# AditMeh/torch-distributed-sandbox

Hardware: AMD Instinct MI355X
Metric: images/sec (whole node), 3000x3000 MNIST ConvNet DDP at 1/2/4/8 MI355X (higher is better)
Workload: dtype fp32 (conv2 fwd+dgrad+wgrad: TF32-class -- one fp16 MFMA per product, both operands rounded to 11 significant bits = TF32's significand, exact power-of-two range scaling, fp32 accumulate: the arithmetic of the reference's default cuDNN TF32 convolutions; conv1 fwd+wgrad: bf16x3 split MFMA (~2^-16)

## Files before the change

torch_distributed_sandbox_amd/csrc/kernels/conv2_fwd2.hip:

```cpp
#include <cstdlib>

#include "bn_finalize.h"
#include "conv2_common.h"
#include "launchers.h"
#include "pooled_layout.h"

namespace tds {

constexpr int F2_TH = 8, F2_TC = 16;
constexpr int F2_SR = F2_TH + 4, F2_SC = F2_TC + 4;
constexpr int F2_REC = F2_SR * F2_SC;
constexpr int F2_THREADS = 256;
constexpr int F2_PGROUPS = 8;
constexpr int F2_PPLANE = F2_PGROUPS * 32 * 32;
constexpr int F2_PBUF = F2_PPLANE;
constexpr int F2_WG = 3;
constexpr int F2_PXREC = 32 * 2 + 16;
constexpr int F2_STAGE = F2_TH * F2_TC * F2_PXREC;
constexpr int F2_OFF_S = 2 * F2_PBUF;
constexpr int F2_YSTAGE = 32 * 32 * 4 + 32 * 2 * 4;
constexpr int F2_OFF_Y = F2_OFF_S + 2 * F2_STAGE;
constexpr int F2_LDS = F2_OFF_Y + 2 * F2_YSTAGE;
constexpr int F2_DMA_PER_WAVE = F2_PGROUPS / (F2_THREADS / 64);
static_assert(F2_LDS % 16 == 0, "LDS carve");
static_assert(F2_WG * F2_LDS <= 160 * 1024, "workgroups per CU");

__device__ __attribute__((aligned(16))) uint32_t g_f2_zero[4] = {0u, 0u, 0u, 0u};

struct F2Tile {
  int b, r0, c0;
};

template <int DIAG, int WV>
__device__ __forceinline__ void f2_dma(const uint4* __restrict__ p1, const F2Tile& x, int P, char* buf, int lane) {
  if constexpr (DIAG == 3) return;
  const char* base = reinterpret_cast<const char*>(p1) + (((int64_t)x.b * P + x.r0 - 2) * P + (x.c0 - 2)) * 32;
#pragma unroll
  for (int j = 0; j < F2_DMA_PER_WAVE; ++j) {
    const int rg = WV * F2_DMA_PER_WAVE + j;
    const int px = rg * 32 + (lane >> 1), half = lane & 1;
    const int rr = px / F2_SC, cc = px - rr * F2_SC;
    const int gr = x.r0 - 2 + rr, gc = x.c0 - 2 + cc;
    const bool ok = px < F2_REC && gr >= 0 && gr < P && gc >= 0 && gc < P;
    const char* src = ok ? base + ((int64_t)rr * P + cc) * 32 + half * 16 : reinterpret_cast<const char*>(g_f2_zero);
    __builtin_amdgcn_global_load_lds(src, (__attribute__((address_space(3))) void*)(buf + rg * 1024), 16, 0, 0);
  }
}

template <int DIAG>
__device__ __forceinline__ void f2_compute(const char* buf, const f32x4 (&W)[13], f32x4 (&acc)[4], int RH, int lane) {
  constexpr int DEPTH = 4;
  const int li = lane & 15, g = lane >> 4;
  const int boff = (g & 1) * 16;
  const char* ph = buf;
#pragma unroll
  for (int o = 0; o < 4; ++o) acc[o] = f32x4{0.f, 0.f, 0.f, 0.f};
  s16x8 ah[DEPTH];
  auto load_a = [&](int i) {
    const int grp = i >> 3, R = i & 7;
    int rec;
    if (grp < 2) {
      rec = (4 * RH + R) * F2_SC + li + 2 * grp + (g >> 1);
    } else {
      int row = 4 * RH + R + (g >> 1);
      if (row > F2_SR - 1) row = F2_SR - 1;
      rec = row * F2_SC + li + 4;
    }
    ah[i % DEPTH] = lds8<DIAG>(ph + rec * 32 + boff);
  };
#pragma unroll
  for (int i = 0; i < DEPTH - 1; ++i) load_a(i);
#pragma unroll
  for (int i = 0; i < 24; ++i) {
    if (i + DEPTH - 1 < 24) load_a(i + DEPTH - 1);
    __builtin_amdgcn_sched_barrier(0);
    const int grp = i >> 3, R = i & 7, cur = i % DEPTH;
    if (grp < 2) {
#pragma unroll
      for (int ky = 0; ky < 5; ++ky) {
        const int o = R - ky;
        if (o >= 0 && o < 4)
          acc[o] = mmaw<DIAG>(ah[cur], __builtin_bit_cast(s16x8, W[2 * ky + grp]), acc[o]);
      }
    } else {
#pragma unroll
      for (int kp = 0; kp < 3; ++kp) {
        const int o = R - 2 * kp;
        if (o >= 0 && o < 4)
          acc[o] = mmaw<DIAG>(ah[cur], __builtin_bit_cast(s16x8, W[10 + kp]), acc[o]);
      }
    }
  }
}

__device__ __forceinline__ int f2_stage_off(int row, int px, int chunk) {
  return (row * F2_TC + px) * F2_PXREC + chunk * 16;
}

__device__ __forceinline__ int f2_ystage_off(int co, int e) { return co * 32 + ((((e >> 2) ^ co) & 7) << 2) + (e & 3); }

__device__ __forceinline__ float f2_ext4(float a, float b, float c, float d, bool neg) {
  const float mx = __builtin_elementwise_maximum(__builtin_elementwise_maximum(a, b), __builtin_elementwise_maximum(c, d));
  const float mn = __builtin_elementwise_minimum(__builtin_elementwise_minimum(a, b), __builtin_elementwise_minimum(c, d));
  return neg ? mn : mx;
}

typedef float f2v __attribute__((ext_vector_type(2)));
template <bool EDGE, bool PLAIN>
__device__ __forceinline__ void f2_stage(const f32x4 (&acc)[4], const F2Tile& x, char* stage, float* ystage, int P,
                                         int RH, int NT, int lane, float bco, float inv, float ksc, bool neg, bool zg,
                                         f2v& s_acc, f2v& q_acc, uint32_t& ymx, uint32_t* __restrict__ a2) {
  const int li = lane & 15, g = lane >> 4;
  const int co = 16 * NT + li;
  float ymf = 0.f;
  uint32_t h[4][4];
#pragma unroll
  for (int o = 0; o < 4; ++o)
#pragma unroll
    for (int r = 0; r < 4; ++r) h[o][r] = f16_bits(acc[o][r] * ksc);
#pragma unroll
  for (int o = 0; o < 4; ++o) {
    const int row = 4 * RH + o;
    const bool rok = !EDGE || x.r0 + row < P;
    if constexpr (EDGE) {
#pragma unroll
      for (int r = 0; r < 4; ++r) {
        const float v = acc[o][r];
        if (rok && x.c0 + 4 * g + r < P) {
          s_acc.x += v;
          q_acc.x += v * v;
          ymx = max(ymx, __float_as_uint(v) & 0x7fffffffu);
        }
      }
    } else {
#pragma unroll
      for (int r = 0; r < 4; r += 2) {
        const f2v v = {acc[o][r], acc[o][r + 1]};
        s_acc += v;
        q_acc = __builtin_elementwise_fma(v, v, q_acc);
        ymf = __builtin_elementwise_maximum(ymf, __builtin_elementwise_maximum(fabsf(v.x), fabsf(v.y)));
      }
    }
  }
  if constexpr (!EDGE) ymx = max(ymx, __float_as_uint(ymf));
  uint64_t cb0[4], cb1[4];
#pragma unroll
  for (int i = 0; i < 2; ++i) {
    uint32_t e[2];
#pragma unroll
    for (int j = 0; j < 2; ++j) {
      const float v0 = acc[2 * i][2 * j], v1 = acc[2 * i][2 * j + 1], v2 = acc[2 * i + 1][2 * j];
      const float v3 = acc[2 * i + 1][2 * j + 1];
      float m;
      if constexpr (PLAIN)
        m = __builtin_elementwise_maximum(__builtin_elementwise_maximum(v0, v1), __builtin_elementwise_maximum(v2, v3));
      else
        m = zg ? v0 : f2_ext4(v0, v1, v2, v3, neg);
      e[j] = f16_bits(m * ksc);
      const uint64_t b0 = __builtin_amdgcn_ballot_w64(v0 == m), b1 = __builtin_amdgcn_ballot_w64(v1 == m),
                     b2 = __builtin_amdgcn_ballot_w64(v2 == m);
      cb0[2 * i + j] = ~b0 & (b1 | ~b2);
      cb1[2 * i + j] = ~b0 & ~b1;
    }
    *reinterpret_cast<uint2*>(ystage + f2_ystage_off(co, (2 * RH + i) * 8 + 2 * g)) = make_uint2(e[0], e[1]);
  }
  {
    uint32_t* ab = reinterpret_cast<uint32_t*>(ystage + 32 * 32);
    const bool upper = g >= 2;
    const uint32_t psel = (g & 1) ? 0x07060302u : 0x05040100u;
    if (li == 0) {
#pragma unroll
      for (int sl = 0; sl < 4; ++sl) {
        const uint32_t w0 = upper ? (uint32_t)(cb0[sl] >> 32) : (uint32_t)cb0[sl];
        const uint32_t w1 = upper ? (uint32_t)(cb1[sl] >> 32) : (uint32_t)cb1[sl];
        ab[((2 * RH + (sl >> 1)) * 8 + 2 * g + (sl & 1)) * 2 + NT] = __builtin_amdgcn_perm(w1, w0, psel);
      }
    }
  }
#pragma unroll
  for (int o = 0; o < 4; ++o)
#pragma unroll
    for (int r = 0; r < 4; ++r)
      *reinterpret_cast<unsigned short*>(stage + (((4 * RH + o) * F2_TC + 4 * g + r) * F2_PXREC) + co * 2) =
          (unsigned short)h[o][r];
}

__device__ __forceinline__ void f2_store_ya(const float* ystage, const F2Tile& x, unsigned short* __restrict__ ya,
                                            const PBGeom& pg) {
  const int tr = x.r0 / F2_TH, tc = x.c0 / F2_TC;
  if (tr >= pg.Q4 || tc >= pg.Q8) return;
  const int e = threadIdx.x, co = e >> 3, part = e & 7;
  const uint4 v = *reinterpret_cast<const uint4*>(ystage + f2_ystage_off(co, part * 4));
  st_stream(reinterpret_cast<uint2*>(ya + ((((int64_t)x.b * 32 + co) * pg.Q4 + tr) * pg.Q8 + tc) * 32 + part * 4),
            make_uint2(__builtin_amdgcn_perm(v.y, v.x, 0x05040100u), __builtin_amdgcn_perm(v.w, v.z, 0x05040100u)));
}

__device__ __forceinline__ void f2_store_a2(const float* ystage, const F2Tile& x, uint32_t* __restrict__ a2, int P) {
  const int e = threadIdx.x, Q = P >> 1;
  const int py = (x.r0 >> 1) + (e >> 3), px = (x.c0 >> 1) + (e & 7);
  if (e < 32 && py < Q && px < Q)
    st_stream(reinterpret_cast<uint2*>(a2 + (((int64_t)x.b * Q + py) * Q + px) * 2),
              reinterpret_cast<const uint2*>(ystage + 32 * 32)[e]);
}

constexpr uint64_t F2_QPX = 0xfeab6732dc894510ull;
template <int DIAG>
__device__ __forceinline__ void f2_store(const char* stage, const F2Tile& x, unsigned short* __restrict__ y2h, int P) {
  if constexpr (DIAG == 4) return;
  const int e = threadIdx.x;
  const int qpx = (int)((F2_QPX >> (4 * ((e >> 2) & 15))) & 15u);
#pragma unroll
  for (int i = 0; i < F2_TH * F2_TC * 4 / F2_THREADS; ++i) {
    const int q = e + F2_THREADS * i;
    const int row = q >> 6, px = qpx, c8 = q & 3;
    const int gr = x.r0 + row, gc = x.c0 + px;
    const uint4 v = *reinterpret_cast<const uint4*>(stage + f2_stage_off(row, px, c8));
    if (gr < P && gc < P)
      st_stream(reinterpret_cast<float4*>(y2h + (((int64_t)x.b * P + gr) * P + gc) * 32 + c8 * 8),
                __builtin_bit_cast(float4, v));
  }
}

template <int DIAG, int WV>
__device__ __forceinline__ void f2_run(const uint4* __restrict__ p1, const uint4* __restrict__ wpack,
                                       const float* __restrict__ bias, const float* __restrict__ gamma,
                                       unsigned short* __restrict__ y2, unsigned short* __restrict__ ya,
                                       uint32_t* __restrict__ a2,
                                       double* __restrict__ partial, uint32_t* __restrict__ ypart,
                                       const uint32_t* __restrict__ scales,
                                       const int* __restrict__ order, int sw, int sk, int B, int P, char* smem) {
  constexpr int NT = WV & 1, RH = WV >> 1;
  const int lane = threadIdx.x & 63, li = lane & 15;
  const int tiles_c = (P + F2_TC - 1) / F2_TC, tiles_r = (P + F2_TH - 1) / F2_TH;
  const int per_img = tiles_c * tiles_r, total = per_img * B;
  const int w = xcd_remap(blockIdx.x, gridDim.x);
  const int* __restrict__ mine = order + w * sw;
  auto decode = [&](int kk) {
    F2Tile x;
    int tr, tc;
    tile_from_order(mine, kk * sk, x.b, tr, tc);
    x.r0 = tr * F2_TH;
    x.c0 = tc * F2_TC;
    return x;
  };
  f32x4 W[13];
#pragma unroll
  for (int s = 0; s < 13; ++s) W[s] = __builtin_bit_cast(f32x4, wpack[(s * 2 + NT) * 64 + lane]);
  const float bco = bias[16 * NT + li];
  const float inv = scales != nullptr ? __uint_as_float(scales[0]) * __uint_as_float(scales[1]) : 1.f;
  const float ksc = scales != nullptr ? __uint_as_float(scales[2]) : 1.f;
  const bool neg = gamma != nullptr && gamma[16 * NT + li] < 0.f;
  const bool zg = gamma != nullptr && gamma[16 * NT + li] == 0.f;
  const bool plain = __builtin_amdgcn_readfirstlane(__builtin_amdgcn_ballot_w64(neg || zg) == 0 ? 1 : 0) != 0;
  const PBGeom pg = pb_geom(P / 2);
  float* ys = reinterpret_cast<float*>(smem + F2_OFF_Y);
  f2v s_acc = {0.f, 0.f}, q_acc = {0.f, 0.f};
  double s_d = 0.0, q_d = 0.0;
  uint32_t ymx = 0u;
  f32x4 acc[4];
  F2Tile prev{0, 0, 0};
  bool have_prev = false;
  int t = w;
  if (t < total) f2_dma<DIAG, WV>(p1, decode(0), P, smem, lane);
  int kk = 0;
  for (; t < total; t += gridDim.x, ++kk) {
    const F2Tile cur = decode(kk);
    __syncthreads();
    if (t + (int)gridDim.x < total) f2_dma<DIAG, WV>(p1, decode(kk + 1), P, smem + ((kk + 1) & 1) * F2_PBUF, lane);
    if (have_prev) {
      f2_store<DIAG>(smem + F2_OFF_S + ((kk + 1) & 1) * F2_STAGE, prev, y2, P);
      f2_store_ya(ys + ((kk + 1) & 1) * (F2_YSTAGE / 4), prev, ya, pg);
      f2_store_a2(ys + ((kk + 1) & 1) * (F2_YSTAGE / 4), prev, a2, P);
    }
    f2_compute<DIAG>(smem + (kk & 1) * F2_PBUF, W, acc, RH, lane);
    if (cur.r0 + F2_TH <= P && cur.c0 + F2_TC <= P && plain)
      f2_stage<false, true>(acc, cur, smem + F2_OFF_S + (kk & 1) * F2_STAGE, ys + (kk & 1) * (F2_YSTAGE / 4), P, RH, NT,
                            lane, bco, inv, ksc, neg, zg, s_acc, q_acc, ymx, a2);
    else if (cur.r0 + F2_TH <= P && cur.c0 + F2_TC <= P)
      f2_stage<false, false>(acc, cur, smem + F2_OFF_S + (kk & 1) * F2_STAGE, ys + (kk & 1) * (F2_YSTAGE / 4), P, RH, NT, lane,
                      bco, inv, ksc, neg, zg, s_acc, q_acc, ymx, a2);
    else
      f2_stage<true, false>(acc, cur, smem + F2_OFF_S + (kk & 1) * F2_STAGE, ys + (kk & 1) * (F2_YSTAGE / 4), P, RH, NT, lane,
                     bco, inv, ksc, neg, zg, s_acc, q_acc, ymx, a2);
    s_d += (double)(s_acc.x + s_acc.y);
    q_d += (double)(q_acc.x + q_acc.y);
    s_acc = f2v{0.f, 0.f};
    q_acc = f2v{0.f, 0.f};
    prev = cur;
    have_prev = true;
  }
  __syncthreads();
  if (have_prev) {
    f2_store<DIAG>(smem + F2_OFF_S + ((kk - 1) & 1) * F2_STAGE, prev, y2, P);
    f2_store_ya(ys + ((kk - 1) & 1) * (F2_YSTAGE / 4), prev, ya, pg);
    f2_store_a2(ys + ((kk - 1) & 1) * (F2_YSTAGE / 4), prev, a2, P);
  }
  ymx = max(ymx, (uint32_t)__shfl_xor((int)ymx, 16, 64));
  ymx = max(ymx, (uint32_t)__shfl_xor((int)ymx, 32, 64));
  double s_sum = s_d, q_sum = q_d;
  s_sum += __shfl_xor(s_sum, 16, 64);
  s_sum += __shfl_xor(s_sum, 32, 64);
  q_sum += __shfl_xor(q_sum, 16, 64);
  q_sum += __shfl_xor(q_sum, 32, 64);
  __syncthreads();
  double* red = reinterpret_cast<double*>(smem);
  uint32_t* yred = reinterpret_cast<uint32_t*>(smem + 4 * 16 * 2 * 8);
  if (lane < 16) {
    red[(WV * 16 + li) * 2 + 0] = s_sum;
    red[(WV * 16 + li) * 2 + 1] = q_sum;
    yred[WV * 16 + li] = ymx;
  }
  __syncthreads();
  if (WV == 0 && lane < 64) {
    const int co = lane >> 1, k = lane & 1, nt = co >> 4, c16 = co & 15;
    const double v = (red[(nt * 16 + c16) * 2 + k] + red[((nt + 2) * 16 + c16) * 2 + k]) * (k ? (double)inv * inv : inv);
    st_agent(partial + ((int64_t)co * gridDim.x + blockIdx.x) * 2 + k, v);
    if (ypart != nullptr && k == 0)
      st_agent(ypart + co * gridDim.x + blockIdx.x,
               __float_as_uint(__uint_as_float(max(yred[nt * 16 + c16], yred[(nt + 2) * 16 + c16])) * inv));
  }
}

constexpr int F2_GROUP = 32;
struct F2Fin {
  uint32_t* sync;
  double* gsum;
  uint32_t* gmax;
  int64_t n;
  const float* beta;
  float eps, momentum;
  float* stats;
  float* running_mean;
  float* running_var;
  int64_t* num_batches;
  float* aff;
  uint32_t* mag;
};

__device__ __forceinline__ void f2_finalize(const F2Fin& fin, const double* __restrict__ partial,
                                            const uint32_t* __restrict__ ypart, const float* __restrict__ bias,
                                            const float* __restrict__ gamma, int* flag) {
  const int nwg = (int)gridDim.x, wg = (int)blockIdx.x, tid = (int)threadIdx.x;
  const int ng = (nwg + F2_GROUP - 1) / F2_GROUP, g = wg / F2_GROUP;
  const int w0 = g * F2_GROUP, w1 = min(nwg, w0 + F2_GROUP);
  double* part = reinterpret_cast<double*>(flag + 4);
  if (!tds_arrive(fin.sync + g, (uint32_t)(w1 - w0), flag)) return;
  const double s = wide_row_sum(partial + (int64_t)w0 * 2, w1 - w0, 64, 2, part, 2 * (int64_t)nwg);
  if (tid < 64) st_agent(fin.gsum + (int64_t)g * 64 + tid, s);
  if (ypart != nullptr && tid < 32) {
    uint32_t v[F2_GROUP];
#pragma unroll
    for (int u = 0; u < F2_GROUP; ++u) v[u] = ypart[(int64_t)tid * nwg + min(w0 + u, w1 - 1)];
    uint32_t m = 0u;
#pragma unroll
    for (int u = 0; u < F2_GROUP; ++u) m = max(m, v[u]);
    st_agent(fin.gmax + g * 32 + tid, m);
  }
  if (!tds_arrive(fin.sync + kSyncWordsPerSite - 1, (uint32_t)ng, flag)) return;
  const double sk = wide_row_sum(fin.gsum, ng, 64, 64, part);
  const uint32_t mx = wide_row_max(fin.gmax, ng, 32, 32, reinterpret_cast<uint32_t*>(part + 128));
  if (tid < 64) part[tid] = sk;
  __syncthreads();
  if (tid < 32) {
    const int co = tid;
    if (co == 0 && fin.num_batches) fin.num_batches[0] += 1;
    bn_finalize_channel(co, 32, part[co * 2], part[co * 2 + 1], fin.n, bias, fin.eps, fin.momentum, gamma, fin.beta,
                        fin.stats, fin.running_mean, fin.running_var, fin.aff);
    if (fin.mag != nullptr && ypart != nullptr) fin.mag[co] = mx;
  }
}

template <int DIAG>
__global__ __launch_bounds__(F2_THREADS, F2_WG) void conv2_fwd2_kernel(const uint4* __restrict__ p1,
                                                                   const uint4* __restrict__ wpack,
                                                                   const float* __restrict__ bias,
                                                                   const float* __restrict__ gamma,
                                                                   unsigned short* __restrict__ y2, unsigned short* __restrict__ ya,
                                                                   uint32_t* __restrict__ a2,
                                                                   double* __restrict__ partial,
                                                                   uint32_t* __restrict__ ypart,
                                                                   const uint32_t* __restrict__ scales,
                                                                   const int* __restrict__ order, int sw, int sk,
                                                                   int B, int P, F2Fin fin) {
  extern __shared__ __attribute__((aligned(16))) char smem[];
  const int wv = __builtin_amdgcn_readfirstlane(threadIdx.x >> 6);
  if (wv == 0) f2_run<DIAG, 0>(p1, wpack, bias, gamma, y2, ya, a2, partial, ypart, scales, order, sw, sk, B, P, smem);
  else if (wv == 1) f2_run<DIAG, 1>(p1, wpack, bias, gamma, y2, ya, a2, partial, ypart, scales, order, sw, sk, B, P, smem);
  else if (wv == 2) f2_run<DIAG, 2>(p1, wpack, bias, gamma, y2, ya, a2, partial, ypart, scales, order, sw, sk, B, P, smem);
  else f2_run<DIAG, 3>(p1, wpack, bias, gamma, y2, ya, a2, partial, ypart, scales, order, sw, sk, B, P, smem);
  if (fin.sync != nullptr) {
    __syncthreads();
    f2_finalize(fin, partial, ypart, bias, gamma, reinterpret_cast<int*>(smem));
  }
}

constexpr int F2I_YSTAGE = 32 * 32 * 4;
constexpr int F2I_OFF_Y = 2 * F2_PBUF;
constexpr int F2I_LDS = F2I_OFF_Y + 2 * F2I_YSTAGE;
static_assert(F2I_LDS % 16 == 0 && F2_WG * F2I_LDS <= 160 * 1024, "LDS carve");

template <bool PLAIN>
__device__ __forceinline__ void f2i_pool(const f32x4 (&acc)[4], float* ystage, int RH, int NT, int lane, float ksc,
                                         bool neg, bool zg) {
  const int li = lane & 15, g = lane >> 4;
  const int co = 16 * NT + li;
#pragma unroll
  for (int i = 0; i < 2; ++i) {
    uint32_t e[2];
#pragma unroll
    for (int j = 0; j < 2; ++j) {
      const float v0 = acc[2 * i][2 * j], v1 = acc[2 * i][2 * j + 1], v2 = acc[2 * i + 1][2 * j];
      const float v3 = acc[2 * i + 1][2 * j + 1];
      float m;
      if constexpr (PLAIN)
        m = __builtin_elementwise_maximum(__builtin_elementwise_maximum(v0, v1), __builtin_elementwise_maximum(v2, v3));
      else
        m = zg ? v0 : f2_ext4(v0, v1, v2, v3, neg);
      e[j] = f16_bits(m * ksc);
    }
    *reinterpret_cast<uint2*>(ystage + f2_ystage_off(co, (2 * RH + i) * 8 + 2 * g)) = make_uint2(e[0], e[1]);
  }
}

template <int WV>
__device__ __forceinline__ void f2i_run(const uint4* __restrict__ p1, const uint4* __restrict__ wpack,
                                        const float* __restrict__ gamma, unsigned short* __restrict__ ya,
                                        const uint32_t* __restrict__ scales, const int* __restrict__ order, int sw,
                                        int sk, int B, int P, char* smem) {
  constexpr int NT = WV & 1, RH = WV >> 1;
  const int lane = threadIdx.x & 63, li = lane & 15;
  const int tiles_c = (P + F2_TC - 1) / F2_TC, tiles_r = (P + F2_TH - 1) / F2_TH;
  const int total = tiles_c * tiles_r * B;
  const int w = xcd_remap(blockIdx.x, gridDim.x);
  const int* __restrict__ mine = order + w * sw;
  auto decode = [&](int kk) {
    F2Tile x;
    int tr, tc;
    tile_from_order(mine, kk * sk, x.b, tr, tc);
    x.r0 = tr * F2_TH;
    x.c0 = tc * F2_TC;
    return x;
  };
  f32x4 W[13];
#pragma unroll
  for (int s = 0; s < 13; ++s) W[s] = __builtin_bit_cast(f32x4, wpack[(s * 2 + NT) * 64 + lane]);
  const float ksc = scales != nullptr ? __uint_as_float(scales[2]) : 1.f;
  const bool neg = gamma != nullptr && gamma[16 * NT + li] < 0.f;
  const bool zg = gamma != nullptr && gamma[16 * NT + li] == 0.f;
  const bool plain = __builtin_amdgcn_readfirstlane(__builtin_amdgcn_ballot_w64(neg || zg) == 0 ? 1 : 0) != 0;
  const PBGeom pg = pb_geom(P / 2);
  float* ys = reinterpret_cast<float*>(smem + F2I_OFF_Y);
  f32x4 acc[4];
  F2Tile prev{0, 0, 0};
  bool have_prev = false;
  int t = w;
  if (t < total) f2_dma<0, WV>(p1, decode(0), P, smem, lane);
  int kk = 0;
  for (; t < total; t += gridDim.x, ++kk) {
    const F2Tile cur = decode(kk);
    __syncthreads();
    if (t + (int)gridDim.x < total) f2_dma<0, WV>(p1, decode(kk + 1), P, smem + ((kk + 1) & 1) * F2_PBUF, lane);
    if (have_prev) f2_store_ya(ys + ((kk + 1) & 1) * (F2I_YSTAGE / 4), prev, ya, pg);
    f2_compute<0>(smem + (kk & 1) * F2_PBUF, W, acc, RH, lane);
    if (plain)
      f2i_pool<true>(acc, ys + (kk & 1) * (F2I_YSTAGE / 4), RH, NT, lane, ksc, neg, zg);
    else
      f2i_pool<false>(acc, ys + (kk & 1) * (F2I_YSTAGE / 4), RH, NT, lane, ksc, neg, zg);
    prev = cur;
    have_prev = true;
  }
  __syncthreads();
  if (have_prev) f2_store_ya(ys + ((kk - 1) & 1) * (F2I_YSTAGE / 4), prev, ya, pg);
}

__global__ __launch_bounds__(F2_THREADS, F2_WG) void conv2_fwd2_inference_kernel(
    const uint4* __restrict__ p1, const uint4* __restrict__ wpack, const float* __restrict__ gamma,
    unsigned short* __restrict__ ya, const uint32_t* __restrict__ scales, const int* __restrict__ order, int sw, int sk,
    int B, int P) {
  extern __shared__ __attribute__((aligned(16))) char smem[];
  const int wv = __builtin_amdgcn_readfirstlane(threadIdx.x >> 6);
  if (wv == 0) f2i_run<0>(p1, wpack, gamma, ya, scales, order, sw, sk, B, P, smem);
  else if (wv == 1) f2i_run<1>(p1, wpack, gamma, ya, scales, order, sw, sk, B, P, smem);
  else if (wv == 2) f2i_run<2>(p1, wpack, gamma, ya, scales, order, sw, sk, B, P, smem);
  else f2i_run<3>(p1, wpack, gamma, ya, scales, order, sw, sk, B, P, smem);
}

}

using namespace tds;

int tds_conv2_fwd2_num_wg() { return F2_WG * tds_conv2_num_wg(); }

void tds_conv2_fwd2_tiles(int P, int* tiles_r, int* tiles_c) {
  *tiles_r = (P + F2_TH - 1) / F2_TH;
  *tiles_c = (P + F2_TC - 1) / F2_TC;
}

#ifdef TDS_DIAG
static int f2_diag_env() {
  const char* e = std::getenv("TDS_CONV2_DIAG");
  return e ? std::atoi(e) : 0;
}
#else
static int f2_diag_env() { return 0; }
#endif

int tds_conv2_fwd2_fin_doubles(int nwg) { return ((nwg + F2_GROUP - 1) / F2_GROUP) * 32 * 2; }
int tds_conv2_fwd2_fin_words(int nwg) { return ((nwg + F2_GROUP - 1) / F2_GROUP) * 32; }

void tds_conv2_fwd2_inference(const void* p1, const short* wp, const float* gamma, unsigned short* ya,
                              const uint32_t* scales, const int* order, int nwg, int sw, int sk, int B, int P,
                              hipStream_t st) {
  hipLaunchKernelGGL(conv2_fwd2_inference_kernel, dim3(nwg), dim3(F2_THREADS), F2I_LDS, st,
                     reinterpret_cast<const uint4*>(p1), reinterpret_cast<const uint4*>(wp), gamma, ya, scales, order, sw,
                     sk, B, P);
  TDS_LAUNCH_CHECK();
}

void tds_conv2_fwd2(const void* p1, const short* wp, const float* bias, const float* gamma, void* y2h, unsigned short* ya,
                    uint32_t* a2, double* partial, uint32_t* ypart, const uint32_t* scales, const int* order, int nwg, int sw, int sk,
                    int B, int P, hipStream_t st, const TdsBnFin* bn) {
  const dim3 grid(nwg), block(F2_THREADS);
  F2Fin fin{};
  if (bn != nullptr) {
    fin.sync = tds_sync_words(kSyncConv2Fwd, st);
    if (fin.sync == nullptr || (nwg + F2_GROUP - 1) / F2_GROUP > WRS_MAXL * 4) {
      tds_launch_fail("conv2_fwd2: in-launch BN2 finalize unavailable (sync words / group count)");
      return;
    }
    fin.gsum = bn->dwork;
    fin.gmax = bn->uwork;
    fin.n = (int64_t)B * P * P;
    fin.beta = bn->beta;
    fin.eps = bn->eps;
    fin.momentum = bn->momentum;
    fin.stats = bn->stats;
    fin.running_mean = bn->running_mean;
    fin.running_var = bn->running_var;
    fin.num_batches = bn->num_batches;
    fin.aff = bn->aff;
    fin.mag = bn->mag;
  }
  unsigned short* y2 = static_cast<unsigned short*>(y2h);
  const uint4* pp = reinterpret_cast<const uint4*>(p1);
  const uint4* w = reinterpret_cast<const uint4*>(wp);
  static bool lds_set = false;
  if (!lds_set) {
    (void)hipFuncSetAttribute(reinterpret_cast<const void*>(conv2_fwd2_kernel<0>),
                              hipFuncAttributeMaxDynamicSharedMemorySize, F2_LDS);
#ifdef TDS_DIAG
    (void)hipFuncSetAttribute(reinterpret_cast<const void*>(conv2_fwd2_kernel<1>), hipFuncAttributeMaxDynamicSharedMemorySize, F2_LDS);
    (void)hipFuncSetAttribute(reinterpret_cast<const void*>(conv2_fwd2_kernel<2>), hipFuncAttributeMaxDynamicSharedMemorySize, F2_LDS);
    (void)hipFuncSetAttribute(reinterpret_cast<const void*>(conv2_fwd2_kernel<3>), hipFuncAttributeMaxDynamicSharedMemorySize, F2_LDS);
    (void)hipFuncSetAttribute(reinterpret_cast<const void*>(conv2_fwd2_kernel<4>), hipFuncAttributeMaxDynamicSharedMemorySize, F2_LDS);
#endif
    lds_set = true;
  }
  switch (f2_diag_env()) {
#ifdef TDS_DIAG
    case 1: hipLaunchKernelGGL(conv2_fwd2_kernel<1>, grid, block, F2_LDS, st, pp, w, bias, gamma, y2, ya, a2, partial, ypart, scales, order, sw, sk, B, P, fin); break;
    case 2: hipLaunchKernelGGL(conv2_fwd2_kernel<2>, grid, block, F2_LDS, st, pp, w, bias, gamma, y2, ya, a2, partial, ypart, scales, order, sw, sk, B, P, fin); break;
    case 3: hipLaunchKernelGGL(conv2_fwd2_kernel<3>, grid, block, F2_LDS, st, pp, w, bias, gamma, y2, ya, a2, partial, ypart, scales, order, sw, sk, B, P, fin); break;
    case 4: hipLaunchKernelGGL(conv2_fwd2_kernel<4>, grid, block, F2_LDS, st, pp, w, bias, gamma, y2, ya, a2, partial, ypart, scales, order, sw, sk, B, P, fin); break;
#endif
    default: hipLaunchKernelGGL(conv2_fwd2_kernel<0>, grid, block, F2_LDS, st, pp, w, bias, gamma, y2, ya, a2, partial, ypart, scales, order, sw, sk, B, P, fin); break;
  }
  TDS_LAUNCH_CHECK();
}
```

Before: 2688.

## Precompute per-lane addresses and streamline tile loop in conv2 forward kernel

Hoists the per-lane DMA, staging and store offsets into a struct computed once per wave, and adds fast paths for interior tiles that skip bounds checks. Tile-order entries are decoded directly with the next entry prefetched, and the loop barrier becomes an explicit vmcnt wait plus syncthreads. The argmax bit packing moves from a single-lane loop to scalar pack and writelane instructions, and the y2h half-precision staging is split into its own function. The aim is to cut per-tile integer address arithmetic and divergent branches, at the cost of more live registers and some inline assembly that depends on the compiler placing values in scalar registers.

```diff
diff --git a/torch_distributed_sandbox_amd/csrc/kernels/conv2_fwd2.hip b/torch_distributed_sandbox_amd/csrc/kernels/conv2_fwd2.hip
--- a/torch_distributed_sandbox_amd/csrc/kernels/conv2_fwd2.hip
+++ b/torch_distributed_sandbox_amd/csrc/kernels/conv2_fwd2.hip
@@ -29,22 +29,77 @@
 
 struct F2Tile {
   int b, r0, c0;
+  bool full;
 };
 
+__device__ __forceinline__ F2Tile f2_tile(int entry, int P) {
+  F2Tile x;
+  x.b = entry >> 24;
+  x.r0 = ((entry >> 12) & 4095) * F2_TH;
+  x.c0 = (entry & 4095) * F2_TC;
+  x.full = x.r0 + F2_TH <= P && x.c0 + F2_TC <= P;
+  return x;
+}
+
+struct F2Lane {
+  uint32_t dma[F2_DMA_PER_WAVE];
+  uint32_t st_lds, st_glb;
+  uint32_t ya_lds;
+  int64_t ya_glb;
+  uint32_t a2_glb;
+};
+
+constexpr uint64_t F2_QPX = 0xfeab6732dc894510ull;
+__device__ __forceinline__ int f2_stage_off(int row, int px, int chunk);
+__device__ __forceinline__ int f2_ystage_off(int co, int e);
+
+template <int WV>
+__device__ __forceinline__ F2Lane f2_lane(int P, const PBGeom& pg, int lane) {
+  F2Lane L;
+#pragma unroll
+  for (int j = 0; j < F2_DMA_PER_WAVE; ++j) {
+    const int px = (WV * F2_DMA_PER_WAVE + j) * 32 + (lane >> 1), half = lane & 1;
+    const int rr = px / F2_SC, cc = px - rr * F2_SC;
+    L.dma[j] = px < F2_REC ? (uint32_t)((rr * P + cc) * 32 + half * 16) : 0u;
+  }
+  const int qpx = (int)((F2_QPX >> (4 * (lane >> 2))) & 15u), c8 = lane & 3;
+  L.st_lds = (uint32_t)f2_stage_off(WV, qpx, c8);
+  L.st_glb = (uint32_t)((WV * P + qpx) * 64 + c8 * 16);
+  const int co = WV * 8 + (lane >> 3), part = lane & 7;
+  L.ya_lds = (uint32_t)f2_ystage_off(co, part * 4);
+  L.ya_glb = (int64_t)co * pg.Q4 * pg.Q8 * 32 + part * 4;
+  L.a2_glb = (uint32_t)(((lane >> 3) * (P >> 1) + (lane & 7)) * 8);
+  return L;
+}
+
 template <int DIAG, int WV>
-__device__ __forceinline__ void f2_dma(const uint4* __restrict__ p1, const F2Tile& x, int P, char* buf, int lane) {
+__device__ __forceinline__ void f2_dma(const uint4* __restrict__ p1, const F2Tile& x, int P, char* buf, int lane,
+                                       const F2Lane& L) {
   if constexpr (DIAG == 3) return;
-  const char* base = reinterpret_cast<const char*>(p1) + (((int64_t)x.b * P + x.r0 - 2) * P + (x.c0 - 2)) * 32;
+  const char* base = reinterpret_cast<const char*>(p1) + ((int64_t)(x.b * P + x.r0 - 2) * P + (x.c0 - 2)) * 32;
+  if (x.r0 >= 2 && x.c0 >= 2 && x.r0 + F2_TH + 2 <= P && x.c0 + F2_TC + 2 <= P) {
+#pragma unroll
+    for (int j = 0; j < F2_DMA_PER_WAVE; ++j)
+      __builtin_amdgcn_global_load_lds(base + L.dma[j],
+                                       (__attribute__((address_space(3))) void*)(buf + (WV * F2_DMA_PER_WAVE + j) * 1024),
+                                       16, 0, 0);
+    return;
+  }
 #pragma unroll
   for (int j = 0; j < F2_DMA_PER_WAVE; ++j) {
     const int rg = WV * F2_DMA_PER_WAVE + j;
-    const int px = rg * 32 + (lane >> 1), half = lane & 1;
+    const int px = rg * 32 + (lane >> 1);
     const int rr = px / F2_SC, cc = px - rr * F2_SC;
     const int gr = x.r0 - 2 + rr, gc = x.c0 - 2 + cc;
     const bool ok = px < F2_REC && gr >= 0 && gr < P && gc >= 0 && gc < P;
-    const char* src = ok ? base + ((int64_t)rr * P + cc) * 32 + half * 16 : reinterpret_cast<const char*>(g_f2_zero);
+    const char* src = ok ? base + L.dma[j] : reinterpret_cast<const char*>(g_f2_zero);
     __builtin_amdgcn_global_load_lds(src, (__attribute__((address_space(3))) void*)(buf + rg * 1024), 16, 0, 0);
   }
+}
+
+__device__ __forceinline__ void f2_tile_barrier() {
+  asm volatile("s_waitcnt vmcnt(0)" ::: "memory");
+  __syncthreads();
 }
 
 template <int DIAG>
@@ -113,11 +168,6 @@
   const int li = lane & 15, g = lane >> 4;
   const int co = 16 * NT + li;
   float ymf = 0.f;
-  uint32_t h[4][4];
-#pragma unroll
-  for (int o = 0; o < 4; ++o)
-#pragma unroll
-    for (int r = 0; r < 4; ++r) h[o][r] = f16_bits(acc[o][r] * ksc);
 #pragma unroll
   for (int o = 0; o < 4; ++o) {
     const int row = 4 * RH + o;
@@ -166,58 +216,75 @@
   }
   {
     uint32_t* ab = reinterpret_cast<uint32_t*>(ystage + 32 * 32);
-    const bool upper = g >= 2;
-    const uint32_t psel = (g & 1) ? 0x07060302u : 0x05040100u;
-    if (li == 0) {
-#pragma unroll
-      for (int sl = 0; sl < 4; ++sl) {
-        const uint32_t w0 = upper ? (uint32_t)(cb0[sl] >> 32) : (uint32_t)cb0[sl];
-        const uint32_t w1 = upper ? (uint32_t)(cb1[sl] >> 32) : (uint32_t)cb1[sl];
-        ab[((2 * RH + (sl >> 1)) * 8 + 2 * g + (sl & 1)) * 2 + NT] = __builtin_amdgcn_perm(w1, w0, psel);
+    uint32_t word = 0u;
+#pragma unroll
+    for (int sl = 0; sl < 4; ++sl)
+#pragma unroll
+      for (int gg = 0; gg < 4; ++gg) {
+        const uint32_t w0 = (uint32_t)(cb0[sl] >> (32 * (gg >> 1))), w1 = (uint32_t)(cb1[sl] >> (32 * (gg >> 1)));
+        uint32_t wd;
+        if (gg & 1) asm("s_pack_hh_b32_b16 %0, %1, %2" : "=s"(wd) : "s"(w0), "s"(w1));
+        else asm("s_pack_ll_b32_b16 %0, %1, %2" : "=s"(wd) : "s"(w0), "s"(w1));
+        asm("v_writelane_b32 %0, %1, %2" : "+v"(word) : "s"(wd), "n"(4 * sl + gg));
       }
-    }
-  }
+    const int sl = (lane >> 2) & 3, gg = lane & 3;
+    if (lane < 16) ab[((2 * RH + (sl >> 1)) * 8 + 2 * gg + (sl & 1)) * 2 + NT] = word;
+  }
+}
+
+__device__ __forceinline__ void f2_stage_y2h(const f32x4 (&acc)[4], char* stage, int RH, int NT, int lane, float ksc) {
+  const int li = lane & 15, g = lane >> 4;
+  const int co = 16 * NT + li;
 #pragma unroll
   for (int o = 0; o < 4; ++o)
 #pragma unroll
     for (int r = 0; r < 4; ++r)
       *reinterpret_cast<unsigned short*>(stage + (((4 * RH + o) * F2_TC + 4 * g + r) * F2_PXREC) + co * 2) =
-          (unsigned short)h[o][r];
+          (unsigned short)f16_bits(acc[o][r] * ksc);
 }
 
 __device__ __forceinline__ void f2_store_ya(const float* ystage, const F2Tile& x, unsigned short* __restrict__ ya,
-                                            const PBGeom& pg) {
+                                            const PBGeom& pg, const F2Lane& L) {
   const int tr = x.r0 / F2_TH, tc = x.c0 / F2_TC;
   if (tr >= pg.Q4 || tc >= pg.Q8) return;
-  const int e = threadIdx.x, co = e >> 3, part = e & 7;
-  const uint4 v = *reinterpret_cast<const uint4*>(ystage + f2_ystage_off(co, part * 4));
-  st_stream(reinterpret_cast<uint2*>(ya + ((((int64_t)x.b * 32 + co) * pg.Q4 + tr) * pg.Q8 + tc) * 32 + part * 4),
+  unsigned short* base = ya + ((int64_t)(x.b * 32 * pg.Q4 + tr) * pg.Q8 + tc) * 32;
+  const uint4 v = *reinterpret_cast<const uint4*>(ystage + L.ya_lds);
+  st_stream(reinterpret_cast<uint2*>(base + L.ya_glb),
             make_uint2(__builtin_amdgcn_perm(v.y, v.x, 0x05040100u), __builtin_amdgcn_perm(v.w, v.z, 0x05040100u)));
 }
 
-__device__ __forceinline__ void f2_store_a2(const float* ystage, const F2Tile& x, uint32_t* __restrict__ a2, int P) {
-  const int e = threadIdx.x, Q = P >> 1;
-  const int py = (x.r0 >> 1) + (e >> 3), px = (x.c0 >> 1) + (e & 7);
-  if (e < 32 && py < Q && px < Q)
-    st_stream(reinterpret_cast<uint2*>(a2 + (((int64_t)x.b * Q + py) * Q + px) * 2),
-              reinterpret_cast<const uint2*>(ystage + 32 * 32)[e]);
-}
-
-constexpr uint64_t F2_QPX = 0xfeab6732dc894510ull;
-template <int DIAG>
-__device__ __forceinline__ void f2_store(const char* stage, const F2Tile& x, unsigned short* __restrict__ y2h, int P) {
+template <int WV>
+__device__ __forceinline__ void f2_store_a2(const float* ystage, const F2Tile& x, uint32_t* __restrict__ a2, int P,
+                                            int lane, const F2Lane& L) {
+  if constexpr (WV != 0) return;
+  const int Q = P >> 1;
+  char* base = reinterpret_cast<char*>(a2) + ((int64_t)(x.b * Q + (x.r0 >> 1)) * Q + (x.c0 >> 1)) * 8;
+  bool ok = lane < 32;
+  if (!x.full) ok = ok && (x.r0 >> 1) + (lane >> 3) < Q && (x.c0 >> 1) + (lane & 7) < Q;
+  if (ok)
+    st_stream(reinterpret_cast<uint2*>(base + L.a2_glb), reinterpret_cast<const uint2*>(ystage + 32 * 32)[lane]);
+}
+
+template <int DIAG, int WV>
+__device__ __forceinline__ void f2_store(const char* stage, const F2Tile& x, unsigned short* __restrict__ y2h, int P,
+                                         int lane, const F2Lane& L) {
   if constexpr (DIAG == 4) return;
-  const int e = threadIdx.x;
-  const int qpx = (int)((F2_QPX >> (4 * ((e >> 2) & 15))) & 15u);
-#pragma unroll
-  for (int i = 0; i < F2_TH * F2_TC * 4 / F2_THREADS; ++i) {
-    const int q = e + F2_THREADS * i;
-    const int row = q >> 6, px = qpx, c8 = q & 3;
-    const int gr = x.r0 + row, gc = x.c0 + px;
-    const uint4 v = *reinterpret_cast<const uint4*>(stage + f2_stage_off(row, px, c8));
-    if (gr < P && gc < P)
-      st_stream(reinterpret_cast<float4*>(y2h + (((int64_t)x.b * P + gr) * P + gc) * 32 + c8 * 8),
-                __builtin_bit_cast(float4, v));
+  constexpr int N = F2_TH * F2_TC * 4 / F2_THREADS, LROW = 4 * F2_TC * F2_PXREC;
+  char* base = reinterpret_cast<char*>(y2h) + ((int64_t)(x.b * P + x.r0) * P + x.c0) * 64;
+  const int64_t rs = (int64_t)P * (4 * 64);
+  const char* src = stage + L.st_lds;
+  if (x.full) {
+#pragma unroll
+    for (int i = 0; i < N; ++i)
+      st_stream(reinterpret_cast<float4*>(base + i * rs + L.st_glb),
+                __builtin_bit_cast(float4, *reinterpret_cast<const uint4*>(src + i * LROW)));
+    return;
+  }
+  const bool cok = x.c0 + (int)((F2_QPX >> (4 * (lane >> 2))) & 15u) < P;
+#pragma unroll
+  for (int i = 0; i < N; ++i) {
+    const uint4 v = *reinterpret_cast<const uint4*>(src + i * LROW);
+    if (x.r0 + WV + 4 * i < P && cok) st_stream(reinterpret_cast<float4*>(base + i * rs + L.st_glb), __builtin_bit_cast(float4, v));
   }
 }
 
@@ -235,14 +302,6 @@
   const int per_img = tiles_c * tiles_r, total = per_img * B;
   const int w = xcd_remap(blockIdx.x, gridDim.x);
   const int* __restrict__ mine = order + w * sw;
-  auto decode = [&](int kk) {
-    F2Tile x;
-    int tr, tc;
-    tile_from_order(mine, kk * sk, x.b, tr, tc);
-    x.r0 = tr * F2_TH;
-    x.c0 = tc * F2_TC;
-    return x;
-  };
   f32x4 W[13];
 #pragma unroll
   for (int s = 0; s < 13; ++s) W[s] = __builtin_bit_cast(f32x4, wpack[(s * 2 + NT) * 64 + lane]);
@@ -258,25 +317,36 @@
   double s_d = 0.0, q_d = 0.0;
   uint32_t ymx = 0u;
   f32x4 acc[4];
-  F2Tile prev{0, 0, 0};
+  const F2Lane L = f2_lane<WV>(P, pg, lane);
+  F2Tile nx{0, 0, 0, false}, prev{0, 0, 0, false};
   bool have_prev = false;
   int t = w;
-  if (t < total) f2_dma<DIAG, WV>(p1, decode(0), P, smem, lane);
+  if (t < total) {
+    nx = f2_tile(mine[0], P);
+    f2_dma<DIAG, WV>(p1, nx, P, smem, lane, L);
+  }
   int kk = 0;
   for (; t < total; t += gridDim.x, ++kk) {
-    const F2Tile cur = decode(kk);
-    __syncthreads();
-    if (t + (int)gridDim.x < total) f2_dma<DIAG, WV>(p1, decode(kk + 1), P, smem + ((kk + 1) & 1) * F2_PBUF, lane);
+    const F2Tile cur = nx;
+    const bool more = t + (int)gridDim.x < total;
+    const int ahead = mine[(more ? kk + 1 : kk) * sk];
+    f2_tile_barrier();
+    asm volatile("" ::"s"(ahead));
+    if (more) {
+      nx = f2_tile(ahead, P);
+      f2_dma<DIAG, WV>(p1, nx, P, smem + ((kk + 1) & 1) * F2_PBUF, lane, L);
+    }
     if (have_prev) {
-      f2_store<DIAG>(smem + F2_OFF_S + ((kk + 1) & 1) * F2_STAGE, prev, y2, P);
-      f2_store_ya(ys + ((kk + 1) & 1) * (F2_YSTAGE / 4), prev, ya, pg);
-      f2_store_a2(ys + ((kk + 1) & 1) * (F2_YSTAGE / 4), prev, a2, P);
+      f2_store<DIAG, WV>(smem + F2_OFF_S + ((kk + 1) & 1) * F2_STAGE, prev, y2, P, lane, L);
+      f2_store_ya(ys + ((kk + 1) & 1) * (F2_YSTAGE / 4), prev, ya, pg, L);
+      f2_store_a2<WV>(ys + ((kk + 1) & 1) * (F2_YSTAGE / 4), prev, a2, P, lane, L);
     }
     f2_compute<DIAG>(smem + (kk & 1) * F2_PBUF, W, acc, RH, lane);
-    if (cur.r0 + F2_TH <= P && cur.c0 + F2_TC <= P && plain)
+    f2_stage_y2h(acc, smem + F2_OFF_S + (kk & 1) * F2_STAGE, RH, NT, lane, ksc);
+    if (cur.full && plain)
       f2_stage<false, true>(acc, cur, smem + F2_OFF_S + (kk & 1) * F2_STAGE, ys + (kk & 1) * (F2_YSTAGE / 4), P, RH, NT,
                             lane, bco, inv, ksc, neg, zg, s_acc, q_acc, ymx, a2);
-    else if (cur.r0 + F2_TH <= P && cur.c0 + F2_TC <= P)
+    else if (cur.full)
       f2_stage<false, false>(acc, cur, smem + F2_OFF_S + (kk & 1) * F2_STAGE, ys + (kk & 1) * (F2_YSTAGE / 4), P, RH, NT, lane,
                       bco, inv, ksc, neg, zg, s_acc, q_acc, ymx, a2);
     else
@@ -291,9 +361,9 @@
   }
   __syncthreads();
   if (have_prev) {
-    f2_store<DIAG>(smem + F2_OFF_S + ((kk - 1) & 1) * F2_STAGE, prev, y2, P);
-    f2_store_ya(ys + ((kk - 1) & 1) * (F2_YSTAGE / 4), prev, ya, pg);
-    f2_store_a2(ys + ((kk - 1) & 1) * (F2_YSTAGE / 4), prev, a2, P);
+    f2_store<DIAG, WV>(smem + F2_OFF_S + ((kk - 1) & 1) * F2_STAGE, prev, y2, P, lane, L);
+    f2_store_ya(ys + ((kk - 1) & 1) * (F2_YSTAGE / 4), prev, ya, pg, L);
+    f2_store_a2<WV>(ys + ((kk - 1) & 1) * (F2_YSTAGE / 4), prev, a2, P, lane, L);
   }
   ymx = max(ymx, (uint32_t)__shfl_xor((int)ymx, 16, 64));
   ymx = max(ymx, (uint32_t)__shfl_xor((int)ymx, 32, 64));
@@ -433,14 +503,6 @@
   const int total = tiles_c * tiles_r * B;
   const int w = xcd_remap(blockIdx.x, gridDim.x);
   const int* __restrict__ mine = order + w * sw;
-  auto decode = [&](int kk) {
-    F2Tile x;
-    int tr, tc;
-    tile_from_order(mine, kk * sk, x.b, tr, tc);
-    x.r0 = tr * F2_TH;
-    x.c0 = tc * F2_TC;
-    return x;
-  };
   f32x4 W[13];
 #pragma unroll
   for (int s = 0; s < 13; ++s) W[s] = __builtin_bit_cast(f32x4, wpack[(s * 2 + NT) * 64 + lane]);
@@ -451,16 +513,26 @@
   const PBGeom pg = pb_geom(P / 2);
   float* ys = reinterpret_cast<float*>(smem + F2I_OFF_Y);
   f32x4 acc[4];
-  F2Tile prev{0, 0, 0};
+  const F2Lane L = f2_lane<WV>(P, pg, lane);
+  F2Tile nx{0, 0, 0, false}, prev{0, 0, 0, false};
   bool have_prev = false;
   int t = w;
-  if (t < total) f2_dma<0, WV>(p1, decode(0), P, smem, lane);
+  if (t < total) {
+    nx = f2_tile(mine[0], P);
+    f2_dma<0, WV>(p1, nx, P, smem, lane, L);
+  }
   int kk = 0;
   for (; t < total; t += gridDim.x, ++kk) {
-    const F2Tile cur = decode(kk);
-    __syncthreads();
-    if (t + (int)gridDim.x < total) f2_dma<0, WV>(p1, decode(kk + 1), P, smem + ((kk + 1) & 1) * F2_PBUF, lane);
-    if (have_prev) f2_store_ya(ys + ((kk + 1) & 1) * (F2I_YSTAGE / 4), prev, ya, pg);
+    const F2Tile cur = nx;
+    const bool more = t + (int)gridDim.x < total;
+    const int ahead = mine[(more ? kk + 1 : kk) * sk];
+    f2_tile_barrier();
+    asm volatile("" ::"s"(ahead));
+    if (more) {
+      nx = f2_tile(ahead, P);
+      f2_dma<0, WV>(p1, nx, P, smem + ((kk + 1) & 1) * F2_PBUF, lane, L);
+    }
+    if (have_prev) f2_store_ya(ys + ((kk + 1) & 1) * (F2I_YSTAGE / 4), prev, ya, pg, L);
     f2_compute<0>(smem + (kk & 1) * F2_PBUF, W, acc, RH, lane);
     if (plain)
       f2i_pool<true>(acc, ys + (kk & 1) * (F2I_YSTAGE / 4), RH, NT, lane, ksc, neg, zg);
@@ -470,7 +542,7 @@
     have_prev = true;
   }
   __syncthreads();
-  if (have_prev) f2_store_ya(ys + ((kk - 1) & 1) * (F2I_YSTAGE / 4), prev, ya, pg);
+  if (have_prev) f2_store_ya(ys + ((kk - 1) & 1) * (F2I_YSTAGE / 4), prev, ya, pg, L);
 }
 
 __global__ __launch_bounds__(F2_THREADS, F2_WG) void conv2_fwd2_inference_kernel(
```

Measured after the change: 2725 (median of 6 runs). +1.4%, better.
